# waicool20/BoofCV

Hardware: AMD Instinct MI355X
Metric: 1080p frames/sec detect+describe+associate (higher is better)
Workload: dtype f32 detect / f64 describe / associate: fp16 MFMA candidate filter + exact fp64 re-score; 1 GPU; batch of 256 1920x1080 GrayF32 per GPU: Fast-Hessian detect + SURF-64 (stable) describe + greedy L2 associate with the next frame; batch_per_gpu=256, width=1920, height=1080, ranks_seen=1

## Files before the change

boofcv_amd/csrc/assoc_mfma.hip:

```cpp
#include "common.h"
#include <cfloat>
#include <cmath>
#include <algorithm>

typedef float f32x16 __attribute__((ext_vector_type(16)));
typedef _Float16 h16x8 __attribute__((ext_vector_type(8)));

struct AssocProblem {
	int srcOff, ns, dstOff, nd;
	int rowBase, colBase;
};
struct AssocBlock {
	int p, row0, row1, col0, col1;
};
struct AssocCand {
	int p, i, j, pad;
	double score;
};

#define C16 1.03e-3f
#define ABS16 2.0e-5f
#define BIG16 60000.0f
#define ROW_CHUNKS 9

__device__ __forceinline__ void waveSyncLds() {
	__builtin_amdgcn_fence(__ATOMIC_RELEASE, "wavefront");
	__builtin_amdgcn_wave_barrier();
	__builtin_amdgcn_fence(__ATOMIC_ACQUIRE, "wavefront");
}

__device__ __forceinline__ int scaleExp(float maxN) {
	if (!(maxN > 0.0f)) return 0;
	int e;
	(void)frexpf(maxN, &e);
	return (e + 1) >> 1;
}

#define PREP_ROWS 8
__global__ __launch_bounds__(256) void k_assoc_norms(const double* __restrict__ D, long long rows, float* __restrict__ nrm, int* __restrict__ flags) {
	const long long row0 = (((long long)blockIdx.x * 256 + threadIdx.x) >> 4) * PREP_ROWS;
	const int part = threadIdx.x & 15;
	if (row0 >= rows) return;
	double2 v0[PREP_ROWS], v1[PREP_ROWS];
#pragma unroll
	for (int q = 0; q < PREP_ROWS; q++) {
		const long long row = min(row0 + q, rows - 1);
		const double2* src = (const double2*)(D + row * 64 + 4 * part);
		v0[q] = src[0]; v1[q] = src[1];
	}
#pragma unroll
	for (int q = 0; q < PREP_ROWS; q++) {
		double s = (v0[q].x * v0[q].x + v0[q].y * v0[q].y) + (v1[q].x * v1[q].x + v1[q].y * v1[q].y);
#pragma unroll
		for (int o = 8; o >= 1; o >>= 1) s += __shfl_xor(s, o, 64);
		if (part == 0 && row0 + q < rows) {
			const float n = (float)s;
			const float nUp = n * (1.0f + 4.0f * 5.9604644775390625e-08f);
			nrm[row0 + q] = nUp;
			if (!(s < 1e30)) atomicOr(&flags[0], 1);
			else if (__float_as_int(nUp) > __hip_atomic_load(&flags[1], __ATOMIC_RELAXED, __HIP_MEMORY_SCOPE_AGENT)) atomicMax(&flags[1], __float_as_int(nUp));
		}
	}
}

typedef _Float16 h16x4 __attribute__((ext_vector_type(4)));
__global__ __launch_bounds__(256) void k_assoc_half(const double* __restrict__ D, long long rows, float* __restrict__ nrm, const int* __restrict__ flags,
													  _Float16* __restrict__ Hrow) {
	const long long row0 = (((long long)blockIdx.x * 256 + threadIdx.x) >> 4) * PREP_ROWS;
	const int part = threadIdx.x & 15;
	if (row0 >= rows) return;
	const int q_ = scaleExp(__int_as_float(flags[1]));
	double2 v0[PREP_ROWS], v1[PREP_ROWS];
#pragma unroll
	for (int q = 0; q < PREP_ROWS; q++) {
		const long long row = min(row0 + q, rows - 1);
		const double2* src = (const double2*)(D + row * 64 + 4 * part);
		v0[q] = src[0]; v1[q] = src[1];
	}
#pragma unroll
	for (int q = 0; q < PREP_ROWS; q++) {
		const long long row = row0 + q;
		if (row >= rows) break;
		_Float16* out = Hrow + row * (ROW_CHUNKS * 8);
		const h16x4 hv = {(_Float16)(float)ldexp(v0[q].x, -q_), (_Float16)(float)ldexp(v0[q].y, -q_), (_Float16)(float)ldexp(v1[q].x, -q_),
						  (_Float16)(float)ldexp(v1[q].y, -q_)};
		*(h16x4*)(out + 4 * part) = hv;
		if (part == 0) {
			const float n = ldexpf(nrm[row], -2 * q_);
			const _Float16 hi = (_Float16)n;
			const _Float16 lo = (_Float16)(n - (float)hi);
			const h16x8 e = {hi, lo, (_Float16)1.0f, (_Float16)1.0f, (_Float16)1.0f, (_Float16)0.0f, (_Float16)0.0f, (_Float16)0.0f};
			*(h16x8*)(out + 64) = e;
			nrm[row] = n;
		}
	}
}

__global__ void k_fill_u32(unsigned int* p, long long n, unsigned int v) {
	const long long i = (long long)blockIdx.x * blockDim.x + threadIdx.x;
	if (i < n) p[i] = v;
}

__global__ void k_assoc_thresholds(const AssocProblem* __restrict__ probs, int count, const float* __restrict__ nrmS, const float* __restrict__ nrmD,
								   const unsigned int* __restrict__ rowKey, const unsigned int* __restrict__ colKey, const int* __restrict__ flags,
								   float* __restrict__ rowThr, float* __restrict__ colThr) {
	const int p = blockIdx.y;
	const AssocProblem P = probs[p];
	const float maxRaw = __int_as_float(flags[1]);
	const float maxN = ldexpf(maxRaw, -2 * scaleExp(maxRaw));
	for (int i = blockIdx.x * blockDim.x + threadIdx.x; i < P.ns + P.nd; i += gridDim.x * blockDim.x) {
		if (i < P.ns) {
			const float band = 2.0f * (C16 * (nrmS[P.srcOff + i] + maxN) + ABS16);
			rowThr[P.rowBase + i] = __uint_as_float(rowKey[P.rowBase + i]) + band;
		} else {
			const int j = i - P.ns;
			const float band = 2.0f * (C16 * (nrmD[P.dstOff + j] + maxN) + ABS16);
			colThr[P.colBase + j] = __uint_as_float(colKey[P.colBase + j]) + band;
		}
	}
}

struct MfmaArgs {
	const uint4* Hs;
	const uint4* Hd;
	const AssocProblem* probs;
	const AssocBlock* blocks;
	unsigned int* rowKey;
	unsigned int* colKey;
	const float* rowThr;
	const float* colThr;
	AssocCand* cand;
	int* counter;
	int cap;
#ifdef BHIP_EXPERIMENTS
	int ablate;
#endif
};

#define CAND_LDS 256

__device__ __noinline__ void candSlow(AssocCand* cand, int* counter, int cap, int p, int rr, int col) {
	const int g = atomicAdd(counter, 1);
	if (g < cap) { AssocCand c; c.p = p; c.i = rr; c.j = col; c.pad = 0; c.score = 0; cand[g] = c; }
}
__device__ __forceinline__ void candAdd(const MfmaArgs& A, int2* buf, int* cnt, bool hit, int p, int rr, int col) {
	if (hit) {
		const int pos = atomicAdd(cnt, 1);
		if (pos < CAND_LDS) buf[pos] = make_int2(rr, col);
		else candSlow(A.cand, A.counter, A.cap, p, rr, col);
	}
}
__device__ __forceinline__ void candFlush(const MfmaArgs& A, const int2* buf, const int* cnt, int p, int lane) {
	waveSyncLds();
	const int n = min(*cnt, CAND_LDS);
	if (n == 0) return;
	int base = 0;
	if (lane == 0) base = atomicAdd(A.counter, n);
	base = __builtin_amdgcn_readfirstlane(base);
	for (int k = lane; k < n; k += 64) {
		if (base + k < A.cap) {
			const int2 v = buf[k];
			AssocCand c; c.p = p; c.i = v.x; c.j = v.y; c.pad = 0; c.score = 0;
			A.cand[base + k] = c;
		}
	}
}

__device__ __forceinline__ h16x8 asHalf8(uint4 v) { return __builtin_bit_cast(h16x8, v); }
__device__ __forceinline__ uint4 extChunk(float n0, float n1, float n2, float n3) {
	const h16x8 h = {(_Float16)n0, (_Float16)n1, (_Float16)n2, (_Float16)n3, (_Float16)1.0f, (_Float16)0.0f, (_Float16)0.0f, (_Float16)0.0f};
	return __builtin_bit_cast(uint4, h);
}

#define STRIP_COLS 384
#define STRIP_TILES (STRIP_COLS / 32)
template <int PASS>
__global__ __launch_bounds__(256, 2) void k_assoc_mfma(MfmaArgs A) {
	__shared__ uint4 tileB[STRIP_TILES][10 * 33];
	__shared__ unsigned int colLds[STRIP_COLS];
	__shared__ float rowThrLds[PASS == 2 ? 4 : 1][64];
	__shared__ int2 candLds[PASS == 2 ? 4 : 1][PASS == 2 ? CAND_LDS : 1];
	__shared__ int candCnt[4];
	const AssocBlock B = A.blocks[blockIdx.x];
	if (B.col0 >= B.col1) return;
	const AssocProblem P = A.probs[B.p];
	const int tid = threadIdx.x;
	const int wave = __builtin_amdgcn_readfirstlane(tid >> 6), lane = tid & 63;
	const int r = lane & 31, h = lane >> 5;
	const int ncol = B.col1 - B.col0;
	const int ntile = (ncol + 31) >> 5;
	int2* candBuf = candLds[PASS == 2 ? wave : 0];
	int* candN = &candCnt[wave];
	if (lane == 0) *candN = 0;

	for (int g0 = tid; g0 < ntile * 32 * ROW_CHUNKS; g0 += 4 * 256) {
		uint4 v[4];
#pragma unroll
		for (int q = 0; q < 4; q++) {
			const int g = g0 + 256 * q;
			const int cl = g / ROW_CHUNKS, ch = g - cl * ROW_CHUNKS;
			if (g < ntile * 32 * ROW_CHUNKS && cl < ncol) {
				v[q] = A.Hd[(long long)(P.dstOff + B.col0 + cl) * ROW_CHUNKS + ch];
				if (ch == 8) { const unsigned int x = v[q].x; v[q].x = v[q].y; v[q].y = x; }
			} else {
				v[q] = ch == 8 ? extChunk(1.0f, 1.0f, BIG16, 0.0f) : make_uint4(0, 0, 0, 0);
			}
		}
#pragma unroll
		for (int q = 0; q < 4; q++) {
			const int g = g0 + 256 * q;
			const int cl = g / ROW_CHUNKS, ch = g - cl * ROW_CHUNKS;
			if (g < ntile * 32 * ROW_CHUNKS) tileB[cl >> 5][ch * 33 + (cl & 31)] = v[q];
		}
	}
	for (int g = tid; g < ntile * 32; g += 256) tileB[g >> 5][9 * 33 + (g & 31)] = make_uint4(0, 0, 0, 0);
	for (int c = tid; c < ntile * 32; c += 256)
		colLds[c] = PASS == 1 ? 0xFFFFFFFFu : (c < ncol ? __float_as_uint(A.colThr[P.colBase + B.col0 + c]) : __float_as_uint(-INFINITY));
	__syncthreads();

	uint4 araw[2][5];
	auto loadA = [&](int rowT) {
#pragma unroll
		for (int t = 0; t < 2; t++) {
			const int row = rowT + 32 * t + r;
			if (row < B.row1) {
				const uint4* src = A.Hs + (long long)(P.srcOff + row) * ROW_CHUNKS;
#pragma unroll
				for (int s = 0; s < 4; s++) araw[t][s] = src[2 * s + h];
				araw[t][4] = h == 0 ? src[8] : make_uint4(0, 0, 0, 0);
			} else {
#pragma unroll
				for (int s = 0; s < 4; s++) araw[t][s] = make_uint4(0, 0, 0, 0);
				araw[t][4] = h == 0 ? extChunk(BIG16, 0.0f, 1.0f, 1.0f) : make_uint4(0, 0, 0, 0);
			}
		}
	};
	if (B.row0 + 64 * wave < B.row1) loadA(B.row0 + 64 * wave);
	for (int rowT = B.row0 + 64 * wave; rowT < B.row1; rowT += 256) {
		h16x8 a[2][5];
#pragma unroll
		for (int t = 0; t < 2; t++) {
#pragma unroll
			for (int s = 0; s < 4; s++) a[t][s] = asHalf8(araw[t][s]) * (_Float16)(-2.0f);
			a[t][4] = asHalf8(araw[t][4]);
		}
		if (rowT + 256 < B.row1 && !BHIP_ABLATE(A, 4)) loadA(rowT + 256);
		unsigned int rowM[32];
#pragma unroll
		for (int k = 0; k < 32; k++) rowM[k] = 0xFFFFFFFFu;
		if (PASS == 2) {
			waveSyncLds();
			rowThrLds[wave][lane] = rowT + lane < B.row1 ? A.rowThr[P.rowBase + rowT + lane] : -INFINITY;
			waveSyncLds();
		}
		for (int ct = 0; ct < ntile; ct += 2) {
			const bool two = ct + 1 < ntile;
			const int cA_ = 32 * ct + r, cB_ = cA_ + 32;
			f32x16 acc[2][2];
#pragma unroll
			for (int t = 0; t < 2; t++)
#pragma unroll
				for (int c = 0; c < 2; c++)
#pragma unroll
					for (int g = 0; g < 16; g++) acc[t][c][g] = (c == 0 || two) ? 0.0f : INFINITY;
#pragma unroll
			for (int s = 0; s < 5 && !BHIP_ABLATE(A, 1); s++) {
				const int ch = s < 4 ? 2 * s + h : 8 + h;
				const h16x8 b0 = asHalf8(tileB[ct][ch * 33 + r]);
				acc[0][0] = __builtin_amdgcn_mfma_f32_32x32x16_f16(a[0][s], b0, acc[0][0], 0, 0, 0);
				acc[1][0] = __builtin_amdgcn_mfma_f32_32x32x16_f16(a[1][s], b0, acc[1][0], 0, 0, 0);
				if (two) {
					const h16x8 b1 = asHalf8(tileB[ct + 1][ch * 33 + r]);
					acc[0][1] = __builtin_amdgcn_mfma_f32_32x32x16_f16(a[0][s], b1, acc[0][1], 0, 0, 0);
					acc[1][1] = __builtin_amdgcn_mfma_f32_32x32x16_f16(a[1][s], b1, acc[1][1], 0, 0, 0);
				}
			}
			if (BHIP_ABLATE(A, 2)) continue;
			if (PASS == 1) {
				unsigned int cA = 0xFFFFFFFFu, cB = 0xFFFFFFFFu;
// ... 83 lines not shown
		atomicMin(&colBest[P.colBase + c->j], bits);
	}
}

__global__ __launch_bounds__(256) void k_assoc_argsel(const AssocProblem* __restrict__ probs, const AssocCand* __restrict__ cand,
														const int* __restrict__ counter, int cap, const unsigned long long* __restrict__ rowBest,
														const unsigned long long* __restrict__ colBest, int* __restrict__ rowArg, int* __restrict__ colArg,
														int* __restrict__ colCnt) {
	const int n = min(*counter, cap);
	for (int t = blockIdx.x * blockDim.x + threadIdx.x; t < n; t += gridDim.x * blockDim.x) {
		const AssocCand c = cand[t];
		const AssocProblem P = probs[c.p];
		const unsigned long long bits = (unsigned long long)__double_as_longlong(c.score);
		if (bits == rowBest[P.rowBase + c.i]) atomicMax(&rowArg[P.rowBase + c.i], c.j);
		if (bits == colBest[P.colBase + c.j]) {
			atomicAdd(&colCnt[P.colBase + c.j], 1);
			atomicMax(&colArg[P.colBase + c.j], c.i);
		}
	}
}

__global__ __launch_bounds__(256) void k_assoc_resolve(const AssocProblem* __restrict__ probs, double maxErr, int backwards,
														 const unsigned long long* __restrict__ rowBest, const int* __restrict__ rowArg,
														 const int* __restrict__ colArg, const int* __restrict__ colCnt, int* __restrict__ pairs,
														 double* __restrict__ fit) {
	const AssocProblem P = probs[blockIdx.y];
	for (int i = blockIdx.x * blockDim.x + threadIdx.x; i < P.ns; i += gridDim.x * blockDim.x) {
		const int m = rowArg[P.rowBase + i];
		const double best = __longlong_as_double((long long)rowBest[P.rowBase + i]);
		int outPair = -1;
		double outFit = maxErr;
		if (m >= 0 && best <= maxErr) {
			outPair = m;
			outFit = best;
			if (backwards) {
				if (!(colArg[P.colBase + m] == i && colCnt[P.colBase + m] == 1)) { outPair = -1; outFit = DBL_MAX; }
			}
		}
		pairs[P.srcOff + i] = outPair;
		fit[P.srcOff + i] = outFit;
	}
}

int bhip_assoc_l2_mfma_batched(bhip_ctx* ctx, AssocMfmaWork& W, const double* dev_src, const double* dev_dst, int count, const long long* srcOff,
								 const int* ns, const long long* dstOff, const int* nd, double maxErr, int backwards, int* dev_pairs, double* dev_fit,
								 int* usedMfma) {
	*usedMfma = 0;
	if (count <= 0) { *usedMfma = 1; return BHIP_OK; }
	std::vector<AssocProblem> probs(count);
	std::vector<AssocBlock> blocks;
	long long maxSrcRow = 0, maxDstRow = 0, rowTotal = 0, colTotal = 0;
	double flopsPerPass = 0;
	for (int p = 0; p < count; p++) {
		if (ns[p] <= 0 || nd[p] <= 0) return BHIP_OK;
		if (srcOff[p] + ns[p] > 0x7fffffffLL || dstOff[p] + nd[p] > 0x7fffffffLL) return BHIP_OK;
		probs[p] = {(int)srcOff[p], ns[p], (int)dstOff[p], nd[p], (int)rowTotal, (int)colTotal};
		maxSrcRow = std::max(maxSrcRow, srcOff[p] + ns[p]);
		maxDstRow = std::max(maxDstRow, dstOff[p] + nd[p]);
		rowTotal += ns[p];
		colTotal += nd[p];
		flopsPerPass += 2.0 * ns[p] * (double)nd[p] * 64;
		if (rowTotal > 0x3fffffffLL || colTotal > 0x3fffffffLL) return BHIP_OK;
	}
	long long strips = 0;
	for (int p = 0; p < count; p++) strips += (nd[p] + STRIP_COLS - 1) / STRIP_COLS;
	int rowSplit = (int)std::max<long long>(1, (1024 + strips - 1) / strips);
	{ const char* e = getenv("BHIP_ASSOC_ROWSPLIT"); if (e && atoi(e) > 0) rowSplit = atoi(e); }
	for (int p = 0; p < count; p++) {
		int chunk = (ns[p] + rowSplit - 1) / rowSplit;
		chunk = std::max(256, ((chunk + 255) / 256) * 256);
		for (int c0 = 0; c0 < nd[p]; c0 += STRIP_COLS)
			for (int r0 = 0; r0 < ns[p]; r0 += chunk) blocks.push_back({p, r0, std::min(ns[p], r0 + chunk), c0, std::min(nd[p], c0 + STRIP_COLS)});
	}
	if (count >= 16) {
		std::vector<AssocBlock> q[8];
		for (const AssocBlock& b : blocks) q[b.p & 7].push_back(b);
		size_t longest = 0;
		for (int x = 0; x < 8; x++) longest = std::max(longest, q[x].size());
		blocks.assign(longest * 8, AssocBlock{0, 0, 0, 0, 0});
		for (int x = 0; x < 8; x++)
			for (size_t k = 0; k < q[x].size(); k++) blocks[k * 8 + x] = q[x][k];
	}
	const bool shared = dev_src == dev_dst;
	const long long rowsS = shared ? std::max(maxSrcRow, maxDstRow) : maxSrcRow;
	const int cap = (int)std::min<long long>(0x3fffffffLL, 8 * (rowTotal + colTotal) + 4096);

	BHIP_TRY(W.Fs.reserve(ctx, (size_t)rowsS * ROW_CHUNKS * 16));
	BHIP_TRY(W.nrmS.reserve(ctx, (size_t)rowsS * 4));
	if (!shared) {
		BHIP_TRY(W.Fd.reserve(ctx, (size_t)maxDstRow * ROW_CHUNKS * 16));
		BHIP_TRY(W.nrmD.reserve(ctx, (size_t)maxDstRow * 4));
	}
	BHIP_TRY(W.probs.reserve(ctx, probs.size() * sizeof(AssocProblem)));
	BHIP_TRY(W.blocks.reserve(ctx, blocks.size() * sizeof(AssocBlock)));
	BHIP_TRY(W.keys.reserve(ctx, (size_t)(rowTotal + colTotal) * 4));
	BHIP_TRY(W.thr.reserve(ctx, (size_t)(rowTotal + colTotal) * 4));
	BHIP_TRY(W.best.reserve(ctx, (size_t)(rowTotal + colTotal) * 8));
	BHIP_TRY(W.args.reserve(ctx, (size_t)(rowTotal + 2 * colTotal) * 4));
	BHIP_TRY(W.cand.reserve(ctx, (size_t)cap * sizeof(AssocCand)));
	BHIP_TRY(W.flags.reserve(ctx, 64));

	hipStream_t st = ctx->stream;
	BHIP_HIP(ctx, hipMemcpyAsync(W.probs.p, probs.data(), probs.size() * sizeof(AssocProblem), hipMemcpyHostToDevice, st));
	BHIP_HIP(ctx, hipMemcpyAsync(W.blocks.p, blocks.data(), blocks.size() * sizeof(AssocBlock), hipMemcpyHostToDevice, st));
	BHIP_HIP(ctx, hipMemsetAsync(W.flags.p, 0, 64, st));
	int* flags = W.flags.as<int>();
	int* counters = flags + 2;
	_Float16* Hs = W.Fs.as<_Float16>();
	float* nS = W.nrmS.as<float>();
	_Float16* Hd = shared ? Hs : W.Fd.as<_Float16>();
	float* nD = shared ? nS : W.nrmD.as<float>();
	{
		ProfScope ps(ctx, "k_assoc_prep", (double)(rowsS + (shared ? 0 : maxDstRow)) * (2 * 64 * 8 + ROW_CHUNKS * 16));
		const unsigned gS = (unsigned)((rowsS + 16 * PREP_ROWS - 1) / (16 * PREP_ROWS)), gD = (unsigned)((maxDstRow + 16 * PREP_ROWS - 1) / (16 * PREP_ROWS));
		hipLaunchKernelGGL(k_assoc_norms, dim3(gS), dim3(256), 0, st, dev_src, rowsS, nS, flags);
		if (!shared) hipLaunchKernelGGL(k_assoc_norms, dim3(gD), dim3(256), 0, st, dev_dst, maxDstRow, nD, flags);
		hipLaunchKernelGGL(k_assoc_half, dim3(gS), dim3(256), 0, st, dev_src, rowsS, nS, flags, Hs);
		if (!shared) hipLaunchKernelGGL(k_assoc_half, dim3(gD), dim3(256), 0, st, dev_dst, maxDstRow, nD, flags, Hd);
	}
	unsigned int* rowKey = W.keys.as<unsigned int>();
	unsigned int* colKey = rowKey + rowTotal;
	float* rowThr = W.thr.as<float>();
	float* colThr = rowThr + rowTotal;
	unsigned long long* rowBest = W.best.as<unsigned long long>();
	unsigned long long* colBest = rowBest + rowTotal;
	int* rowArg = W.args.as<int>();
	int* colArg = rowArg + rowTotal;
	int* colCnt = colArg + colTotal;
	const long long nk = rowTotal + colTotal;
	hipLaunchKernelGGL(k_fill_u32, dim3((unsigned)((nk + 255) / 256)), dim3(256), 0, st, rowKey, nk, 0xFFFFFFFFu);
	BHIP_HIP(ctx, hipMemsetAsync(W.best.p, 0xFF, (size_t)nk * 8, st));
	BHIP_HIP(ctx, hipMemsetAsync(rowArg, 0xFF, (size_t)(rowTotal + colTotal) * 4, st));
	BHIP_HIP(ctx, hipMemsetAsync(colCnt, 0, (size_t)colTotal * 4, st));

	MfmaArgs A;
	A.Hs = (const uint4*)Hs; A.Hd = (const uint4*)Hd; A.probs = W.probs.as<AssocProblem>(); A.blocks = W.blocks.as<AssocBlock>();
	A.rowKey = rowKey; A.colKey = colKey; A.rowThr = rowThr; A.colThr = colThr;
	A.cand = W.cand.as<AssocCand>(); A.counter = counters; A.cap = cap;
#ifdef BHIP_EXPERIMENTS
	{ const char* e = getenv("BHIP_ASSOC_ABLATE"); A.ablate = e ? atoi(e) : 0; }
#endif
	const unsigned nblocks = (unsigned)blocks.size();
	{
		ProfScope ps(ctx, "k_assoc_mfma_pass1", 0, flopsPerPass);
		hipLaunchKernelGGL(k_assoc_mfma<1>, dim3(nblocks), dim3(256), 0, st, A);
	}
	int maxN = 0;
	for (int p = 0; p < count; p++) maxN = std::max(maxN, ns[p] + nd[p]);
	hipLaunchKernelGGL(k_assoc_thresholds, dim3((maxN + 255) / 256, count), dim3(256), 0, st, A.probs, count, nS, nD, rowKey, colKey, flags, rowThr, colThr);
	{
		ProfScope ps(ctx, "k_assoc_mfma_pass2", 0, flopsPerPass);
		hipLaunchKernelGGL(k_assoc_mfma<2>, dim3(nblocks), dim3(256), 0, st, A);
	}
	{
		ProfScope ps(ctx, "k_assoc_exact");
		const unsigned exactBlocks = (unsigned)std::min<long long>(16384, std::max<long long>(256, (3 * (rowTotal + colTotal) / 2 + 255) / 256));
		hipLaunchKernelGGL(k_assoc_exact, dim3(exactBlocks), dim3(256), 0, st, dev_src, dev_dst, A.probs, A.cand, counters, cap, rowBest, colBest);
		hipLaunchKernelGGL(k_assoc_argsel, dim3(exactBlocks), dim3(256), 0, st, A.probs, A.cand, counters, cap, rowBest, colBest, rowArg, colArg, colCnt);
	}
	BHIP_HIP(ctx, hipMemcpyAsync(ctx->hostScratch.p, flags, 16, hipMemcpyDeviceToHost, st));
	BHIP_HIP(ctx, hipStreamSynchronize(st));
	const int* hf = ctx->hostScratch.as<int>();
	if (hf[0] != 0 || hf[2] > cap) return BHIP_OK;
	int maxNs = 0;
	for (int p = 0; p < count; p++) maxNs = std::max(maxNs, ns[p]);
	hipLaunchKernelGGL(k_assoc_resolve, dim3((maxNs + 255) / 256, count), dim3(256), 0, st, A.probs, maxErr, backwards, rowBest, rowArg, colArg, colCnt,
					   dev_pairs, dev_fit);
	BHIP_HIP(ctx, hipGetLastError());
	*usedMfma = 1;
	return BHIP_OK;
}
```

boofcv_amd/csrc/cabi.hip:

```cpp
#include "cabi.h"

HandleRegistry& registry() {
	static HandleRegistry* r = [] {
		HandleRegistry* p = new HandleRegistry();
		atexit([] { registry().exiting = true; });
		return p;
	}();
	return *r;
}

static int ctxCreate(int device, void* stream, bool useGiven, bhip_ctx** out) {
	if (!out) return BHIP_ERR_INVALID;
	*out = nullptr;
	int count = 0;
	if (hipGetDeviceCount(&count) != hipSuccess || count <= 0) return BHIP_ERR_HIP;
	if (device < 0 || device >= count) return BHIP_ERR_INVALID;
	if (hipSetDevice(device) != hipSuccess) return BHIP_ERR_HIP;
	std::unique_ptr<bhip_ctx_full> ctx(new (std::nothrow) bhip_ctx_full());
	if (!ctx) return BHIP_ERR_NOMEM;
	ctx->device = device;
	if (hipDeviceGetAttribute(&ctx->cuCount, hipDeviceAttributeMultiprocessorCount, device) != hipSuccess || ctx->cuCount <= 0) return BHIP_ERR_HIP;
	if (useGiven) {
		ctx->stream = (hipStream_t)stream;
	} else {
// ... 15 lines not shown
struct FhOctavePlan {
	int skip, w, h, nlevels;
	int sizes[BHIP_MAX_LEVELS];
	std::vector<FhLevelPlan> mids;
	bool fused = false, fixed = false;
	int shareFrom[BHIP_MAX_LEVELS];
	bool onDemand[BHIP_MAX_LEVELS];
	int exportSlot[BHIP_MAX_LEVELS];
	int nexport = 0;
	size_t intenOff = 0, expOff = 0;
	long long intenImageStride = 0, expImageStride = 0;
};

struct FhDetector {
	bhip_fh_cfg cfg;
	int W = 0, H = 0, batch = 0, cap = 0;
	bool plannedInt = false;
	std::vector<FhOctavePlan> plan;
	int bitmapWords = 0;
	DevBuf inten, bitmap, prefix, cand, sorted, count, selKey, selIdx, selLevels;
	bool nBest() const { return cfg.maxFeaturesPerScale > 0; }
	std::vector<int> counts;
	long long total = 0;

	static bool unfusedOnly() { return bhip_env_flag("BHIP_DETECT_UNFUSED"); }
	int makePlan(bhip_ctx* ctx, int width, int height) {
		plan.clear();
		if (cfg.numberScalesPerOctave > BHIP_MAX_LEVELS || cfg.numberScalesPerOctave < 1) return bhip_fail(ctx, BHIP_ERR_UNSUPPORTED, "numberScalesPerOctave out of range");
		if (cfg.extractRadius < 1) return bhip_fail(ctx, BHIP_ERR_INVALID, "Search radius must be >= 1");
		if (cfg.initialSampleSize < 1 || cfg.initialSize < 3) return bhip_fail(ctx, BHIP_ERR_INVALID, "bad sample size / initial size");
		if (width >= 32768 || height >= 32768) return bhip_fail(ctx, BHIP_ERR_UNSUPPORTED, "image too large for Point2D_I16");
		int skip = cfg.initialSampleSize, sizeStep = cfg.scaleStepSize, octaveSize = cfg.initialSize;
		unsigned int bits = 0;
		const int step = cfg.extractRadius + 1;
		for (int octave = 0; octave < cfg.numberOfOctaves; octave++) {
			FhOctavePlan o;
			o.nlevels = cfg.numberScalesPerOctave;
			for (int i = 0; i < o.nlevels; i++) o.sizes[i] = octaveSize + i * sizeStep;
			const int maxSize = o.sizes[o.nlevels - 1];
			if (maxSize > width || maxSize > height) break;
			o.skip = skip;
			o.w = width / skip;
			o.h = height / skip;
			for (int i = 2; i < o.nlevels; i++) {
				FhLevelPlan m;
				m.level = i - 1;
// ... 142 lines not shown
					FusedExport ex{0, {0, 0}, nullptr, 0, 0, 0, {0, 0}};
					if (o.nexport > 0 && k + 1 < plan.size()) {
						const FhOctavePlan& c = plan[k + 1];
						ex.n = o.nexport;
						for (int j = 0; j < o.nlevels; j++) if (o.exportSlot[j] >= 0) ex.level[o.exportSlot[j]] = j;
						ex.out = level(c, 0).data; ex.w = c.w; ex.h = c.h; ex.imageStride = c.intenImageStride;
						for (int i = 0; i < c.nlevels; i++) {
							const int j = c.shareFrom[i];
							if (j >= 0 && o.exportSlot[j] >= 0) ex.slotOffset[o.exportSlot[j]] = (long long)i * c.w * c.h;
						}
					}
					BHIP_TRY(bhip_launch_detect_fused(ctx, ii, o.skip, o.nlevels, o.sizes, (int)o.mids.size(), mp, ml, cfg.extractRadius,
													  cfg.detectThreshold, bitmap.as<unsigned int>(), bitmapWords, cand.as<KeyPoint>(), count.as<int>(), cap,
													  ex.n > 0 ? &ex : nullptr));
					continue;
				}
				size_t end = k + 1;
				while (!nBest() && end < plan.size() && !plan[end].fused) end++;
				BHIP_TRY(runStandAlone(ctx, ii, k, end));
				k = end - 1;
			}
			BHIP_TRY(bhip_launch_word_prefix(ctx, bitmap.as<unsigned int>(), bitmapWords, batch, prefix.as<unsigned int>(), count.as<int>() + batch));
			counts.resize(batch);
			if ((size_t)batch * 4 <= (1u << 20)) {
				BHIP_HIP(ctx, hipMemcpyAsync(ctx->hostScratch.p, count.p, (size_t)batch * 4, hipMemcpyDeviceToHost, ctx->stream));
				BHIP_HIP(ctx, hipStreamSynchronize(ctx->stream));
				memcpy(counts.data(), ctx->hostScratch.p, (size_t)batch * 4);
			} else {
				BHIP_HIP(ctx, hipMemcpyAsync(counts.data(), count.p, (size_t)batch * 4, hipMemcpyDeviceToHost, ctx->stream));
				BHIP_HIP(ctx, hipStreamSynchronize(ctx->stream));
			}
			int maxCount = 0;
			total = 0;
			for (int c : counts) { maxCount = std::max(maxCount, c); total += c; }
			if (maxCount <= cap) {
				BHIP_TRY(bhip_launch_rank_scatter(ctx, bitmap.as<unsigned int>(), bitmapWords, prefix.as<unsigned int>(), cand.as<KeyPoint>(), count.as<int>(),
												  cap, batch, sorted.as<KeyPoint>()));
				if (nBest()) BHIP_TRY(selectNBest(ctx));
				return BHIP_OK;
			}
			cap = maxCount + maxCount / 4 + 64;
			BHIP_TRY(allocate(ctx));
		}
		return bhip_fail(ctx, BHIP_ERR_CAPACITY, "key point list kept overflowing");
	}
	int selectNBest(bhip_ctx* ctx) {
		int nlv = 0;
		for (auto& o : plan) nlv += (int)o.mids.size();
		int* levelStart = selLevels.as<int>();
		int* levelCount = levelStart + (size_t)std::max(nlv, 1) * batch;
		int li = 0;
		for (auto& o : plan)
			for (auto& m : o.mids) {
				BHIP_TRY(bhip_launch_select_nbest(ctx, level(o, m.level - 1), level(o, m.level), level(o, m.level + 1), m.p, cfg.extractRadius,
												  cfg.maxFeaturesPerScale, bitmap.as<unsigned int>(), prefix.as<unsigned int>(), bitmapWords, sorted.as<KeyPoint>(),
												  cap, selKey.as<float>(), selIdx.as<int>(), cand.as<KeyPoint>(), levelStart, levelCount, li, nlv));
				li++;
			}
		BHIP_TRY(bhip_launch_compact_levels(ctx, cand.as<KeyPoint>(), cap, levelStart, levelCount, nlv, batch, sorted.as<KeyPoint>(), count.as<int>()));
		BHIP_HIP(ctx, hipMemcpyAsync(counts.data(), count.p, (size_t)batch * 4, hipMemcpyDeviceToHost, ctx->stream));
		BHIP_HIP(ctx, hipStreamSynchronize(ctx->stream));
// ... 698 lines not shown
```

boofcv_amd/csrc/common.h:

```cpp
#pragma once
#include <hip/hip_runtime.h>
#include <cstdint>
#include <cstdio>
#include <cstring>
#include <cstdlib>
#include <string>
#include <type_traits>
#include <vector>
#include <new>
#include <utility>
#include "../../include/boofhip.h"

#define BHIP_WAVE 64

static inline bool bhip_env_flag(const char* name) {
	const char* e = getenv(name);
	return e && e[0] == '1';
}
#ifdef BHIP_EXPERIMENTS
#define BHIP_ABLATE(P, bits) ((P).ablate & (bits))
#else
#define BHIP_ABLATE(P, bits) 0
#endif

// ... 73 lines not shown
	DevBuf(DevBuf&& o) noexcept : p(o.p), cap(o.cap) { o.p = nullptr; o.cap = 0; }
	DevBuf& operator=(DevBuf&& o) noexcept { std::swap(p, o.p); std::swap(cap, o.cap); return *this; }
	~DevBuf() { if (p) (void)hipFree(p); }
	int reserve(bhip_ctx* ctx, size_t bytes) {
		if (bytes <= cap) return BHIP_OK;
		if (p) { BHIP_HIP(ctx, hipStreamSynchronize(ctx->stream)); BHIP_HIP(ctx, hipFree(p)); p = nullptr; cap = 0; }
		size_t want = bytes + bytes / 8;
		BHIP_HIP(ctx, hipMalloc(&p, want));
		cap = want;
		return BHIP_OK;
	}
	template <class T> T* as() const { return (T*)p; }
};

inline int PinnedBuf::reserve(bhip_ctx* ctx, size_t bytes) {
	if (bytes <= cap) return BHIP_OK;
	if (p) { BHIP_HIP(ctx, hipStreamSynchronize(ctx->stream)); (void)hipHostFree(p); p = nullptr; cap = 0; }
	if (hipHostMalloc(&p, bytes, hipHostMallocDefault) != hipSuccess) { (void)hipGetLastError(); p = nullptr; return bhip_fail(ctx, BHIP_ERR_NOMEM, "page-locked staging buffer"); }
	cap = bytes;
	return BHIP_OK;
}

struct AssocMfmaWork {
	DevBuf Fs, Fd, nrmS, nrmD, probs, blocks, keys, thr, best, args, cand, flags;
};

struct ImgView {
	const float* data;
	long long imageStride;
	int stride;
	int width, height;
};
struct ImgViewW {
	float* data;
	long long imageStride;
	int stride;
	int width, height;
};

template <class T>
struct DevImg {
	T* data;
	long long imageStride;
	int stride, width, height, batch;
	operator DevImg<const T>() const { return {data, imageStride, stride, width, height, batch}; }
};
template <class T>
// ... 380 lines not shown
```

boofcv_amd/csrc/detect.hip:

```cpp
#include "hessian_dev.h"
#include <cfloat>

template <bool MIN> __device__ __forceinline__ bool nmsBeats(float a, float b) { return MIN ? a <= b : a >= b; }
template <bool MIN> __device__ __forceinline__ float nmsPad() { return MIN ? INFINITY : -INFINITY; }
template <bool MIN> __device__ __forceinline__ float nmsMarker() { return MIN ? -FLT_MAX : FLT_MAX; }
template <int RT, bool MIN = false>
__device__ __forceinline__ bool strictLocalMax(const float* __restrict__ img, int stride, int w, int h, int x, int y, int r, float v, float thr) {
	if (!nmsBeats<MIN>(v, thr) || v == nmsMarker<MIN>()) return false;
	bool isMax = true;
	if (RT > 0) {
		float nb[(2 * RT + 1) * (2 * RT + 1)];
#pragma unroll
		for (int j = -RT; j <= RT; j++)
#pragma unroll
			for (int i = -RT; i <= RT; i++) {
				const int xx = x + i, yy = y + j;
				const bool in = xx >= 0 && xx < w && yy >= 0 && yy < h && !(i == 0 && j == 0);
				nb[(j + RT) * (2 * RT + 1) + i + RT] = in ? img[(long long)yy * stride + xx] : nmsPad<MIN>();
			}
#pragma unroll
		for (int k = 0; k < (2 * RT + 1) * (2 * RT + 1); k++)
			if (nmsBeats<MIN>(nb[k], v)) isMax = false;
	} else {
		const int x0 = max(x - r, 0), x1 = min(x + r, w - 1), y0 = max(y - r, 0), y1 = min(y + r, h - 1);
// ... 330 lines not shown
}

int bhip_launch_word_prefix(bhip_ctx* ctx, const unsigned int* bitmap, int bitmapWords, int batch, unsigned int* wordPrefix, int* totals) {
	if (batch <= 0 || bitmapWords <= 0) return BHIP_OK;
	{
		ProfScope ps(ctx, "k_word_prefix", 8.0 * bitmapWords * batch);
		hipLaunchKernelGGL(k_word_prefix, dim3(batch), dim3(1024), 0, ctx->stream, bitmap, bitmapWords, wordPrefix, totals);
	}
	BHIP_HIP(ctx, hipGetLastError());
	return BHIP_OK;
}

__global__ __launch_bounds__(256) void k_rank_scatter(const unsigned int* __restrict__ bitmap, int words, const unsigned int* __restrict__ prefix,
													   const KeyPoint* __restrict__ cand, const int* __restrict__ candCount, int cap,
													   KeyPoint* __restrict__ sorted) {
	const int img = blockIdx.y;
	const int n = min(candCount[img], cap);
	const int i = blockIdx.x * blockDim.x + threadIdx.x;
	if (i >= n) return;
	const KeyPoint kp = cand[(long long)img * cap + i];
	const unsigned int word = kp.key >> 5, bit = kp.key & 31;
	const unsigned int below = bitmap[(long long)img * words + word] & ((1u << bit) - 1u);
	const unsigned int rank = prefix[(long long)img * words + word] + __popc(below);
	sorted[(long long)img * cap + rank] = kp;
}

int bhip_launch_rank_scatter(bhip_ctx* ctx, const unsigned int* bitmap, int bitmapWords, unsigned int* wordPrefix, const KeyPoint* cand,
							 const int* candCount, int cap, int batch, KeyPoint* sorted) {
	if (batch <= 0 || cap <= 0) return BHIP_OK;
	dim3 grid((cap + 255) / 256, batch);
	{
		ProfScope ps(ctx, "k_rank_scatter");
		hipLaunchKernelGGL(k_rank_scatter, grid, dim3(256), 0, ctx->stream, bitmap, bitmapWords, (const unsigned int*)wordPrefix, cand, candCount, cap, sorted);
	}
	BHIP_HIP(ctx, hipGetLastError());
	return BHIP_OK;
}

#define SEL_LDS 4096

struct SelectParams {
	const float* lower;
	const float* mid;
	const float* upper;
	long long imageStride;
	int stride;
	DetectLevelParams p;
// ... 385 lines not shown
```

Before: 16190 frames/s.

## Speculate fp16 scale from previous call and fold assoc prep/init launches

The association path now guesses the fp16 scaling exponent from the previous call. This lets norms and fp16 conversion fuse into one prep kernel, and the result is validated afterwards, re-running the whole association if the guess was wrong. Memsets, fills and host-to-device table copies are folded into a single init kernel that copies the tables from pinned host memory. The threshold kernel is removed by computing thresholds inside pass 2, and resolve is launched before the host sync and gated on device flags. Detection overlaps rank-scatter with the count readback, the MFMA loop peels the odd tail tile, and a mispredicted scale costs a full second run.

```diff
diff --git a/boofcv_amd/csrc/assoc_mfma.hip b/boofcv_amd/csrc/assoc_mfma.hip
--- a/boofcv_amd/csrc/assoc_mfma.hip
+++ b/boofcv_amd/csrc/assoc_mfma.hip
@@ -1,6 +1,7 @@
 #include "common.h"
 #include <cfloat>
 #include <cmath>
+#include <cstring>
 #include <algorithm>
 
 typedef float f32x16 __attribute__((ext_vector_type(16)));
@@ -29,11 +30,22 @@
 	__builtin_amdgcn_fence(__ATOMIC_ACQUIRE, "wavefront");
 }
 
-__device__ __forceinline__ int scaleExp(float maxN) {
+__host__ __device__ __forceinline__ int scaleExp(float maxN) {
 	if (!(maxN > 0.0f)) return 0;
 	int e;
 	(void)frexpf(maxN, &e);
 	return (e + 1) >> 1;
+}
+__host__ __device__ __forceinline__ bool scaleHolds(float maxN, int q) {
+	if (!(maxN > 0.0f)) return true;
+	int e;
+	(void)frexpf(maxN, &e);
+	return e >= 2 * q - 3 && e <= 2 * q;
+}
+__host__ __device__ __forceinline__ bool assocDegenerate(const int* flags, int cap) {
+	float maxN;
+	memcpy(&maxN, &flags[1], 4);
+	return flags[0] != 0 || flags[2] > cap || !scaleHolds(maxN, flags[3]);
 }
 
 #define PREP_ROWS 8
@@ -64,12 +76,13 @@
 }
 
 typedef _Float16 h16x4 __attribute__((ext_vector_type(4)));
-__global__ __launch_bounds__(256) void k_assoc_half(const double* __restrict__ D, long long rows, float* __restrict__ nrm, const int* __restrict__ flags,
+__global__ __launch_bounds__(256) void k_assoc_half(const double* __restrict__ D, long long rows, float* __restrict__ nrm, int* __restrict__ flags,
 													  _Float16* __restrict__ Hrow) {
 	const long long row0 = (((long long)blockIdx.x * 256 + threadIdx.x) >> 4) * PREP_ROWS;
 	const int part = threadIdx.x & 15;
 	if (row0 >= rows) return;
 	const int q_ = scaleExp(__int_as_float(flags[1]));
+	if (blockIdx.x == 0 && threadIdx.x == 0) flags[3] = q_;
 	double2 v0[PREP_ROWS], v1[PREP_ROWS];
 #pragma unroll
 	for (int q = 0; q < PREP_ROWS; q++) {
@@ -96,28 +109,55 @@
 	}
 }
 
-__global__ void k_fill_u32(unsigned int* p, long long n, unsigned int v) {
-	const long long i = (long long)blockIdx.x * blockDim.x + threadIdx.x;
-	if (i < n) p[i] = v;
-}
-
-__global__ void k_assoc_thresholds(const AssocProblem* __restrict__ probs, int count, const float* __restrict__ nrmS, const float* __restrict__ nrmD,
-								   const unsigned int* __restrict__ rowKey, const unsigned int* __restrict__ colKey, const int* __restrict__ flags,
-								   float* __restrict__ rowThr, float* __restrict__ colThr) {
-	const int p = blockIdx.y;
-	const AssocProblem P = probs[p];
-	const float maxRaw = __int_as_float(flags[1]);
-	const float maxN = ldexpf(maxRaw, -2 * scaleExp(maxRaw));
-	for (int i = blockIdx.x * blockDim.x + threadIdx.x; i < P.ns + P.nd; i += gridDim.x * blockDim.x) {
-		if (i < P.ns) {
-			const float band = 2.0f * (C16 * (nrmS[P.srcOff + i] + maxN) + ABS16);
-			rowThr[P.rowBase + i] = __uint_as_float(rowKey[P.rowBase + i]) + band;
-		} else {
-			const int j = i - P.ns;
-			const float band = 2.0f * (C16 * (nrmD[P.dstOff + j] + maxN) + ABS16);
-			colThr[P.colBase + j] = __uint_as_float(colKey[P.colBase + j]) + band;
-		}
-	}
+__global__ __launch_bounds__(256) void k_assoc_prep_hinted(const double* __restrict__ D, long long rows, int q_, float* __restrict__ nrm, int* __restrict__ flags,
+															 _Float16* __restrict__ Hrow) {
+	const long long row0 = (((long long)blockIdx.x * 256 + threadIdx.x) >> 4) * PREP_ROWS;
+	const int part = threadIdx.x & 15;
+	if (row0 >= rows) return;
+	double2 v0[PREP_ROWS], v1[PREP_ROWS];
+#pragma unroll
+	for (int q = 0; q < PREP_ROWS; q++) {
+		const long long row = min(row0 + q, rows - 1);
+		const double2* src = (const double2*)(D + row * 64 + 4 * part);
+		v0[q] = src[0]; v1[q] = src[1];
+	}
+#pragma unroll
+	for (int q = 0; q < PREP_ROWS; q++) {
+		double s = (v0[q].x * v0[q].x + v0[q].y * v0[q].y) + (v1[q].x * v1[q].x + v1[q].y * v1[q].y);
+#pragma unroll
+		for (int o = 8; o >= 1; o >>= 1) s += __shfl_xor(s, o, 64);
+		const long long row = row0 + q;
+		if (row >= rows) continue;
+		_Float16* out = Hrow + row * (ROW_CHUNKS * 8);
+		const h16x4 hv = {(_Float16)(float)ldexp(v0[q].x, -q_), (_Float16)(float)ldexp(v0[q].y, -q_), (_Float16)(float)ldexp(v1[q].x, -q_),
+						  (_Float16)(float)ldexp(v1[q].y, -q_)};
+		*(h16x4*)(out + 4 * part) = hv;
+		if (part == 0) {
+			const float nRaw = (float)s;
+			const float nUp = nRaw * (1.0f + 4.0f * 5.9604644775390625e-08f);
+			if (!(s < 1e30)) atomicOr(&flags[0], 1);
+			else if (__float_as_int(nUp) > __hip_atomic_load(&flags[1], __ATOMIC_RELAXED, __HIP_MEMORY_SCOPE_AGENT)) atomicMax(&flags[1], __float_as_int(nUp));
+			const float n = ldexpf(nUp, -2 * q_);
+			const _Float16 hi = (_Float16)n;
+			const _Float16 lo = (_Float16)(n - (float)hi);
+			const h16x8 e = {hi, lo, (_Float16)1.0f, (_Float16)1.0f, (_Float16)1.0f, (_Float16)0.0f, (_Float16)0.0f, (_Float16)0.0f};
+			*(h16x8*)(out + 64) = e;
+			nrm[row] = n;
+		}
+	}
+}
+
+__global__ __launch_bounds__(256) void k_assoc_init(unsigned int* __restrict__ keys, unsigned long long* __restrict__ best, int* __restrict__ args, long long nk,
+													  long long colTotal, int* __restrict__ flags, int q_, const uint4* __restrict__ tabSrc, uint4* __restrict__ tabDst,
+													  long long tabWords) {
+	const long long i = (long long)blockIdx.x * 256 + threadIdx.x;
+	if (i < tabWords) tabDst[i] = tabSrc[i];
+	if (i < 16) flags[i] = i == 3 ? q_ : 0;
+	if (i >= nk) return;
+	keys[i] = 0xFFFFFFFFu;
+	best[i] = ~0ull;
+	args[i] = -1;
+	if (i < colTotal) args[nk + i] = 0;
 }
 
 struct MfmaArgs {
@@ -127,8 +167,9 @@
 	const AssocBlock* blocks;
 	unsigned int* rowKey;
 	unsigned int* colKey;
-	const float* rowThr;
-	const float* colThr;
+	const float* nrmS;
+	const float* nrmD;
+	const int* flags;
 	AssocCand* cand;
 	int* counter;
 	int cap;
@@ -172,6 +213,9 @@
 	return __builtin_bit_cast(uint4, h);
 }
 
+#ifndef BHIP_ASSOC_PEEL
+#define BHIP_ASSOC_PEEL 1
+#endif
 #define STRIP_COLS 384
 #define STRIP_TILES (STRIP_COLS / 32)
 template <int PASS>
@@ -214,8 +258,20 @@
 		}
 	}
 	for (int g = tid; g < ntile * 32; g += 256) tileB[g >> 5][9 * 33 + (g & 31)] = make_uint4(0, 0, 0, 0);
-	for (int c = tid; c < ntile * 32; c += 256)
-		colLds[c] = PASS == 1 ? 0xFFFFFFFFu : (c < ncol ? __float_as_uint(A.colThr[P.colBase + B.col0 + c]) : __float_as_uint(-INFINITY));
+	float maxN = 0.0f;
+	if (PASS == 2) maxN = ldexpf(__int_as_float(A.flags[1]), -2 * A.flags[3]);
+	for (int c = tid; c < ntile * 32; c += 256) {
+		unsigned int v = 0xFFFFFFFFu;
+		if (PASS == 2) {
+			float thr = -INFINITY;
+			if (c < ncol) {
+				const float band = 2.0f * (C16 * (A.nrmD[P.dstOff + B.col0 + c] + maxN) + ABS16);
+				thr = __uint_as_float(A.colKey[P.colBase + B.col0 + c]) + band;
+			}
+			v = __float_as_uint(thr);
+		}
+		colLds[c] = v;
+	}
 	__syncthreads();
 
 	uint4 araw[2][5];
@@ -250,11 +306,18 @@
 		for (int k = 0; k < 32; k++) rowM[k] = 0xFFFFFFFFu;
 		if (PASS == 2) {
 			waveSyncLds();
-			rowThrLds[wave][lane] = rowT + lane < B.row1 ? A.rowThr[P.rowBase + rowT + lane] : -INFINITY;
+			float thr = -INFINITY;
+			if (rowT + lane < B.row1) {
+				const float band = 2.0f * (C16 * (A.nrmS[P.srcOff + rowT + lane] + maxN) + ABS16);
+				thr = __uint_as_float(A.rowKey[P.rowBase + rowT + lane]) + band;
+			}
+			rowThrLds[wave][lane] = thr;
 			waveSyncLds();
 		}
-		for (int ct = 0; ct < ntile; ct += 2) {
-			const bool two = ct + 1 < ntile;
+#pragma unroll
+		for (int round = 0; round <= BHIP_ASSOC_PEEL; round++)
+		for (int ct = round == 0 ? 0 : (ntile & ~1); ct < (BHIP_ASSOC_PEEL && round == 0 ? (ntile & ~1) : ntile); ct += 2) {
+			const bool two = BHIP_ASSOC_PEEL ? round == 0 : ct + 1 < ntile;
 			const int cA_ = 32 * ct + r, cB_ = cA_ + 32;
 			f32x16 acc[2][2];
 #pragma unroll
@@ -384,8 +447,9 @@
 
 __global__ __launch_bounds__(256) void k_assoc_resolve(const AssocProblem* __restrict__ probs, double maxErr, int backwards,
 														 const unsigned long long* __restrict__ rowBest, const int* __restrict__ rowArg,
-														 const int* __restrict__ colArg, const int* __restrict__ colCnt, int* __restrict__ pairs,
-														 double* __restrict__ fit) {
+														 const int* __restrict__ colArg, const int* __restrict__ colCnt, const int* __restrict__ flags, int cap,
+														 int* __restrict__ pairs, double* __restrict__ fit) {
+	if (assocDegenerate(flags, cap)) return;
 	const AssocProblem P = probs[blockIdx.y];
 	for (int i = blockIdx.x * blockDim.x + threadIdx.x; i < P.ns; i += gridDim.x * blockDim.x) {
 		const int m = rowArg[P.rowBase + i];
@@ -424,25 +488,27 @@
 		flopsPerPass += 2.0 * ns[p] * (double)nd[p] * 64;
 		if (rowTotal > 0x3fffffffLL || colTotal > 0x3fffffffLL) return BHIP_OK;
 	}
-	long long strips = 0;
-	for (int p = 0; p < count; p++) strips += (nd[p] + STRIP_COLS - 1) / STRIP_COLS;
-	int rowSplit = (int)std::max<long long>(1, (1024 + strips - 1) / strips);
-	{ const char* e = getenv("BHIP_ASSOC_ROWSPLIT"); if (e && atoi(e) > 0) rowSplit = atoi(e); }
-	for (int p = 0; p < count; p++) {
-		int chunk = (ns[p] + rowSplit - 1) / rowSplit;
-		chunk = std::max(256, ((chunk + 255) / 256) * 256);
-		for (int c0 = 0; c0 < nd[p]; c0 += STRIP_COLS)
-			for (int r0 = 0; r0 < ns[p]; r0 += chunk) blocks.push_back({p, r0, std::min(ns[p], r0 + chunk), c0, std::min(nd[p], c0 + STRIP_COLS)});
-	}
-	if (count >= 16) {
-		std::vector<AssocBlock> q[8];
-		for (const AssocBlock& b : blocks) q[b.p & 7].push_back(b);
-		size_t longest = 0;
-		for (int x = 0; x < 8; x++) longest = std::max(longest, q[x].size());
-		blocks.assign(longest * 8, AssocBlock{0, 0, 0, 0, 0});
-		for (int x = 0; x < 8; x++)
-			for (size_t k = 0; k < q[x].size(); k++) blocks[k * 8 + x] = q[x][k];
-	}
+	auto buildBlocks = [&]() {
+		long long strips = 0;
+		for (int p = 0; p < count; p++) strips += (nd[p] + STRIP_COLS - 1) / STRIP_COLS;
+		int rowSplit = (int)std::max<long long>(1, (1024 + strips - 1) / strips);
+		{ const char* e = getenv("BHIP_ASSOC_ROWSPLIT"); if (e && atoi(e) > 0) rowSplit = atoi(e); }
+		for (int p = 0; p < count; p++) {
+			int chunk = (ns[p] + rowSplit - 1) / rowSplit;
+			chunk = std::max(256, ((chunk + 255) / 256) * 256);
+			for (int c0 = 0; c0 < nd[p]; c0 += STRIP_COLS)
+				for (int r0 = 0; r0 < ns[p]; r0 += chunk) blocks.push_back({p, r0, std::min(ns[p], r0 + chunk), c0, std::min(nd[p], c0 + STRIP_COLS)});
+		}
+		if (count >= 16) {
+			std::vector<AssocBlock> q[8];
+			for (const AssocBlock& b : blocks) q[b.p & 7].push_back(b);
+			size_t longest = 0;
+			for (int x = 0; x < 8; x++) longest = std::max(longest, q[x].size());
+			blocks.assign(longest * 8, AssocBlock{0, 0, 0, 0, 0});
+			for (int x = 0; x < 8; x++)
+				for (size_t k = 0; k < q[x].size(); k++) blocks[k * 8 + x] = q[x][k];
+		}
+	};
 	const bool shared = dev_src == dev_dst;
 	const long long rowsS = shared ? std::max(maxSrcRow, maxDstRow) : maxSrcRow;
 	const int cap = (int)std::min<long long>(0x3fffffffLL, 8 * (rowTotal + colTotal) + 4096);
@@ -453,82 +519,102 @@
 		BHIP_TRY(W.Fd.reserve(ctx, (size_t)maxDstRow * ROW_CHUNKS * 16));
 		BHIP_TRY(W.nrmD.reserve(ctx, (size_t)maxDstRow * 4));
 	}
-	BHIP_TRY(W.probs.reserve(ctx, probs.size() * sizeof(AssocProblem)));
-	BHIP_TRY(W.blocks.reserve(ctx, blocks.size() * sizeof(AssocBlock)));
 	BHIP_TRY(W.keys.reserve(ctx, (size_t)(rowTotal + colTotal) * 4));
-	BHIP_TRY(W.thr.reserve(ctx, (size_t)(rowTotal + colTotal) * 4));
 	BHIP_TRY(W.best.reserve(ctx, (size_t)(rowTotal + colTotal) * 8));
 	BHIP_TRY(W.args.reserve(ctx, (size_t)(rowTotal + 2 * colTotal) * 4));
 	BHIP_TRY(W.cand.reserve(ctx, (size_t)cap * sizeof(AssocCand)));
 	BHIP_TRY(W.flags.reserve(ctx, 64));
 
 	hipStream_t st = ctx->stream;
-	BHIP_HIP(ctx, hipMemcpyAsync(W.probs.p, probs.data(), probs.size() * sizeof(AssocProblem), hipMemcpyHostToDevice, st));
-	BHIP_HIP(ctx, hipMemcpyAsync(W.blocks.p, blocks.data(), blocks.size() * sizeof(AssocBlock), hipMemcpyHostToDevice, st));
-	BHIP_HIP(ctx, hipMemsetAsync(W.flags.p, 0, 64, st));
 	int* flags = W.flags.as<int>();
 	int* counters = flags + 2;
 	_Float16* Hs = W.Fs.as<_Float16>();
 	float* nS = W.nrmS.as<float>();
 	_Float16* Hd = shared ? Hs : W.Fd.as<_Float16>();
 	float* nD = shared ? nS : W.nrmD.as<float>();
-	{
-		ProfScope ps(ctx, "k_assoc_prep", (double)(rowsS + (shared ? 0 : maxDstRow)) * (2 * 64 * 8 + ROW_CHUNKS * 16));
-		const unsigned gS = (unsigned)((rowsS + 16 * PREP_ROWS - 1) / (16 * PREP_ROWS)), gD = (unsigned)((maxDstRow + 16 * PREP_ROWS - 1) / (16 * PREP_ROWS));
-		hipLaunchKernelGGL(k_assoc_norms, dim3(gS), dim3(256), 0, st, dev_src, rowsS, nS, flags);
-		if (!shared) hipLaunchKernelGGL(k_assoc_norms, dim3(gD), dim3(256), 0, st, dev_dst, maxDstRow, nD, flags);
-		hipLaunchKernelGGL(k_assoc_half, dim3(gS), dim3(256), 0, st, dev_src, rowsS, nS, flags, Hs);
-		if (!shared) hipLaunchKernelGGL(k_assoc_half, dim3(gD), dim3(256), 0, st, dev_dst, maxDstRow, nD, flags, Hd);
-	}
 	unsigned int* rowKey = W.keys.as<unsigned int>();
 	unsigned int* colKey = rowKey + rowTotal;
-	float* rowThr = W.thr.as<float>();
-	float* colThr = rowThr + rowTotal;
 	unsigned long long* rowBest = W.best.as<unsigned long long>();
 	unsigned long long* colBest = rowBest + rowTotal;
 	int* rowArg = W.args.as<int>();
 	int* colArg = rowArg + rowTotal;
 	int* colCnt = colArg + colTotal;
 	const long long nk = rowTotal + colTotal;
-	hipLaunchKernelGGL(k_fill_u32, dim3((unsigned)((nk + 255) / 256)), dim3(256), 0, st, rowKey, nk, 0xFFFFFFFFu);
-	BHIP_HIP(ctx, hipMemsetAsync(W.best.p, 0xFF, (size_t)nk * 8, st));
-	BHIP_HIP(ctx, hipMemsetAsync(rowArg, 0xFF, (size_t)(rowTotal + colTotal) * 4, st));
-	BHIP_HIP(ctx, hipMemsetAsync(colCnt, 0, (size_t)colTotal * 4, st));
+	int maxNs = 0;
+	for (int p = 0; p < count; p++) maxNs = std::max(maxNs, ns[p]);
+	const size_t blocksAt = (probs.size() * sizeof(AssocProblem) + 15) & ~(size_t)15;
 
 	MfmaArgs A;
-	A.Hs = (const uint4*)Hs; A.Hd = (const uint4*)Hd; A.probs = W.probs.as<AssocProblem>(); A.blocks = W.blocks.as<AssocBlock>();
-	A.rowKey = rowKey; A.colKey = colKey; A.rowThr = rowThr; A.colThr = colThr;
+	A.Hs = (const uint4*)Hs; A.Hd = (const uint4*)Hd;
+	A.rowKey = rowKey; A.colKey = colKey; A.nrmS = nS; A.nrmD = nD; A.flags = flags;
 	A.cand = W.cand.as<AssocCand>(); A.counter = counters; A.cap = cap;
 #ifdef BHIP_EXPERIMENTS
 	{ const char* e = getenv("BHIP_ASSOC_ABLATE"); A.ablate = e ? atoi(e) : 0; }
 #endif
+	const unsigned gS = (unsigned)((rowsS + 16 * PREP_ROWS - 1) / (16 * PREP_ROWS)), gD = (unsigned)((maxDstRow + 16 * PREP_ROWS - 1) / (16 * PREP_ROWS));
+	const double prepRows = (double)(rowsS + (shared ? 0 : maxDstRow));
+
+	buildBlocks();
+	const size_t tableBytes = (blocksAt + blocks.size() * sizeof(AssocBlock) + 15) & ~(size_t)15;
+	BHIP_TRY(W.probs.reserve(ctx, tableBytes));
+	if (W.tablesInFlight) { BHIP_HIP(ctx, hipStreamSynchronize(st)); W.tablesInFlight = false; }
+	if (tableBytes > W.tables.cap) BHIP_TRY(W.tables.reserve(ctx, tableBytes * 2));
+	memcpy(W.tables.p, probs.data(), probs.size() * sizeof(AssocProblem));
+	memcpy((char*)W.tables.p + blocksAt, blocks.data(), blocks.size() * sizeof(AssocBlock));
+	void* tablesDev = nullptr;
+	BHIP_HIP(ctx, hipHostGetDevicePointer(&tablesDev, W.tables.p, 0));
+	if (!W.flagsRead) BHIP_HIP(ctx, hipEventCreateWithFlags(&W.flagsRead.h, hipEventDisableTiming));
+	A.probs = W.probs.as<AssocProblem>();
+	A.blocks = (const AssocBlock*)((const char*)W.probs.p + blocksAt);
 	const unsigned nblocks = (unsigned)blocks.size();
-	{
-		ProfScope ps(ctx, "k_assoc_mfma_pass1", 0, flopsPerPass);
-		hipLaunchKernelGGL(k_assoc_mfma<1>, dim3(nblocks), dim3(256), 0, st, A);
-	}
-	int maxN = 0;
-	for (int p = 0; p < count; p++) maxN = std::max(maxN, ns[p] + nd[p]);
-	hipLaunchKernelGGL(k_assoc_thresholds, dim3((maxN + 255) / 256, count), dim3(256), 0, st, A.probs, count, nS, nD, rowKey, colKey, flags, rowThr, colThr);
-	{
-		ProfScope ps(ctx, "k_assoc_mfma_pass2", 0, flopsPerPass);
-		hipLaunchKernelGGL(k_assoc_mfma<2>, dim3(nblocks), dim3(256), 0, st, A);
-	}
-	{
-		ProfScope ps(ctx, "k_assoc_exact");
-		const unsigned exactBlocks = (unsigned)std::min<long long>(16384, std::max<long long>(256, (3 * (rowTotal + colTotal) / 2 + 255) / 256));
-		hipLaunchKernelGGL(k_assoc_exact, dim3(exactBlocks), dim3(256), 0, st, dev_src, dev_dst, A.probs, A.cand, counters, cap, rowBest, colBest);
-		hipLaunchKernelGGL(k_assoc_argsel, dim3(exactBlocks), dim3(256), 0, st, A.probs, A.cand, counters, cap, rowBest, colBest, rowArg, colArg, colCnt);
-	}
-	BHIP_HIP(ctx, hipMemcpyAsync(ctx->hostScratch.p, flags, 16, hipMemcpyDeviceToHost, st));
-	BHIP_HIP(ctx, hipStreamSynchronize(st));
-	const int* hf = ctx->hostScratch.as<int>();
-	if (hf[0] != 0 || hf[2] > cap) return BHIP_OK;
-	int maxNs = 0;
-	for (int p = 0; p < count; p++) maxNs = std::max(maxNs, ns[p]);
-	hipLaunchKernelGGL(k_assoc_resolve, dim3((maxNs + 255) / 256, count), dim3(256), 0, st, A.probs, maxErr, backwards, rowBest, rowArg, colArg, colCnt,
-					   dev_pairs, dev_fit);
-	BHIP_HIP(ctx, hipGetLastError());
-	*usedMfma = 1;
+
+	for (int run = 0; run < 2; run++) {
+		const bool hinted = run == 0;
+		const long long tabWords = hinted ? (long long)(tableBytes / 16) : 0;
+		W.tablesInFlight = true;
+		hipLaunchKernelGGL(k_assoc_init, dim3((unsigned)((std::max(nk, tabWords) + 255) / 256)), dim3(256), 0, st, rowKey, rowBest, rowArg, nk, colTotal, flags,
+						   hinted ? W.scaleHint : 0, (const uint4*)tablesDev, W.probs.as<uint4>(), tabWords);
+		if (hinted) {
+			ProfScope ps(ctx, "k_assoc_prep", prepRows * (64 * 8 + ROW_CHUNKS * 16));
+			hipLaunchKernelGGL(k_assoc_prep_hinted, dim3(gS), dim3(256), 0, st, dev_src, rowsS, W.scaleHint, nS, flags, Hs);
+			if (!shared) hipLaunchKernelGGL(k_assoc_prep_hinted, dim3(gD), dim3(256), 0, st, dev_dst, maxDstRow, W.scaleHint, nD, flags, Hd);
+		} else {
+			ProfScope ps(ctx, "k_assoc_prep", prepRows * (2 * 64 * 8 + ROW_CHUNKS * 16));
+			hipLaunchKernelGGL(k_assoc_norms, dim3(gS), dim3(256), 0, st, dev_src, rowsS, nS, flags);
+			if (!shared) hipLaunchKernelGGL(k_assoc_norms, dim3(gD), dim3(256), 0, st, dev_dst, maxDstRow, nD, flags);
+			hipLaunchKernelGGL(k_assoc_half, dim3(gS), dim3(256), 0, st, dev_src, rowsS, nS, flags, Hs);
+			if (!shared) hipLaunchKernelGGL(k_assoc_half, dim3(gD), dim3(256), 0, st, dev_dst, maxDstRow, nD, flags, Hd);
+		}
+		{
+			ProfScope ps(ctx, "k_assoc_mfma_pass1", 0, flopsPerPass);
+			hipLaunchKernelGGL(k_assoc_mfma<1>, dim3(nblocks), dim3(256), 0, st, A);
+		}
+		{
+			ProfScope ps(ctx, "k_assoc_mfma_pass2", 0, flopsPerPass);
+			hipLaunchKernelGGL(k_assoc_mfma<2>, dim3(nblocks), dim3(256), 0, st, A);
+		}
+		{
+			ProfScope ps(ctx, "k_assoc_exact");
+			const unsigned exactBlocks = (unsigned)std::min<long long>(16384, std::max<long long>(256, (3 * (rowTotal + colTotal) / 2 + 255) / 256));
+			hipLaunchKernelGGL(k_assoc_exact, dim3(exactBlocks), dim3(256), 0, st, dev_src, dev_dst, A.probs, A.cand, counters, cap, rowBest, colBest);
+			hipLaunchKernelGGL(k_assoc_argsel, dim3(exactBlocks), dim3(256), 0, st, A.probs, A.cand, counters, cap, rowBest, colBest, rowArg, colArg, colCnt);
+		}
+		BHIP_HIP(ctx, hipMemcpyAsync(ctx->hostScratch.p, flags, 16, hipMemcpyDeviceToHost, st));
+		BHIP_HIP(ctx, hipEventRecord(W.flagsRead, st));
+		hipLaunchKernelGGL(k_assoc_resolve, dim3((maxNs + 255) / 256, count), dim3(256), 0, st, A.probs, maxErr, backwards, rowBest, rowArg, colArg, colCnt,
+						   flags, cap, dev_pairs, dev_fit);
+		BHIP_HIP(ctx, hipEventSynchronize(W.flagsRead));
+		W.tablesInFlight = false;
+		BHIP_HIP(ctx, hipGetLastError());
+		const int* hf = ctx->hostScratch.as<int>();
+		if (hf[0] != 0) return BHIP_OK;
+		float maxRaw;
+		memcpy(&maxRaw, &hf[1], 4);
+		if (maxRaw > 0.0f) W.scaleHint = scaleExp(maxRaw);
+		if (!scaleHolds(maxRaw, hf[3])) continue;
+		if (hf[2] > cap) return BHIP_OK;
+		*usedMfma = 1;
+		return BHIP_OK;
+	}
 	return BHIP_OK;
 }
diff --git a/boofcv_amd/csrc/cabi.hip b/boofcv_amd/csrc/cabi.hip
--- a/boofcv_amd/csrc/cabi.hip
+++ b/boofcv_amd/csrc/cabi.hip
@@ -61,6 +61,7 @@
 	bool nBest() const { return cfg.maxFeaturesPerScale > 0; }
 	std::vector<int> counts;
 	long long total = 0;
+	HipEvent countsRead;
 
 	static bool unfusedOnly() { return bhip_env_flag("BHIP_DETECT_UNFUSED"); }
 	int makePlan(bhip_ctx* ctx, int width, int height) {
@@ -249,21 +250,27 @@
 			}
 			BHIP_TRY(bhip_launch_word_prefix(ctx, bitmap.as<unsigned int>(), bitmapWords, batch, prefix.as<unsigned int>(), count.as<int>() + batch));
 			counts.resize(batch);
-			if ((size_t)batch * 4 <= (1u << 20)) {
-				BHIP_HIP(ctx, hipMemcpyAsync(ctx->hostScratch.p, count.p, (size_t)batch * 4, hipMemcpyDeviceToHost, ctx->stream));
-				BHIP_HIP(ctx, hipStreamSynchronize(ctx->stream));
-				memcpy(counts.data(), ctx->hostScratch.p, (size_t)batch * 4);
+			const bool viaScratch = (size_t)batch * 4 <= (1u << 20);
+			BHIP_HIP(ctx, hipMemcpyAsync(viaScratch ? ctx->hostScratch.p : (void*)counts.data(), count.p, (size_t)batch * 4, hipMemcpyDeviceToHost, ctx->stream));
+			if (!nBest()) {
+				if (!countsRead) BHIP_HIP(ctx, hipEventCreateWithFlags(&countsRead.h, hipEventDisableTiming));
+				BHIP_HIP(ctx, hipEventRecord(countsRead, ctx->stream));
+				BHIP_TRY(bhip_launch_rank_scatter(ctx, bitmap.as<unsigned int>(), bitmapWords, prefix.as<unsigned int>(), cand.as<KeyPoint>(), count.as<int>(),
+												  cap, batch, sorted.as<KeyPoint>()));
+				BHIP_HIP(ctx, hipEventSynchronize(countsRead));
 			} else {
-				BHIP_HIP(ctx, hipMemcpyAsync(counts.data(), count.p, (size_t)batch * 4, hipMemcpyDeviceToHost, ctx->stream));
 				BHIP_HIP(ctx, hipStreamSynchronize(ctx->stream));
 			}
+			if (viaScratch) memcpy(counts.data(), ctx->hostScratch.p, (size_t)batch * 4);
 			int maxCount = 0;
 			total = 0;
 			for (int c : counts) { maxCount = std::max(maxCount, c); total += c; }
 			if (maxCount <= cap) {
-				BHIP_TRY(bhip_launch_rank_scatter(ctx, bitmap.as<unsigned int>(), bitmapWords, prefix.as<unsigned int>(), cand.as<KeyPoint>(), count.as<int>(),
-												  cap, batch, sorted.as<KeyPoint>()));
-				if (nBest()) BHIP_TRY(selectNBest(ctx));
+				if (nBest()) {
+					BHIP_TRY(bhip_launch_rank_scatter(ctx, bitmap.as<unsigned int>(), bitmapWords, prefix.as<unsigned int>(), cand.as<KeyPoint>(), count.as<int>(),
+													  cap, batch, sorted.as<KeyPoint>()));
+					BHIP_TRY(selectNBest(ctx));
+				}
 				return BHIP_OK;
 			}
 			cap = maxCount + maxCount / 4 + 64;
diff --git a/boofcv_amd/csrc/common.h b/boofcv_amd/csrc/common.h
--- a/boofcv_amd/csrc/common.h
+++ b/boofcv_amd/csrc/common.h
@@ -119,7 +119,11 @@
 }
 
 struct AssocMfmaWork {
-	DevBuf Fs, Fd, nrmS, nrmD, probs, blocks, keys, thr, best, args, cand, flags;
+	DevBuf Fs, Fd, nrmS, nrmD, probs, keys, best, args, cand, flags;
+	PinnedBuf tables;
+	bool tablesInFlight = false;
+	HipEvent flagsRead;
+	int scaleHint = 1;
 };
 
 struct ImgView {
diff --git a/boofcv_amd/csrc/detect.hip b/boofcv_amd/csrc/detect.hip
--- a/boofcv_amd/csrc/detect.hip
+++ b/boofcv_amd/csrc/detect.hip
@@ -376,7 +376,7 @@
 	const unsigned int word = kp.key >> 5, bit = kp.key & 31;
 	const unsigned int below = bitmap[(long long)img * words + word] & ((1u << bit) - 1u);
 	const unsigned int rank = prefix[(long long)img * words + word] + __popc(below);
-	sorted[(long long)img * cap + rank] = kp;
+	if (rank < (unsigned int)cap) sorted[(long long)img * cap + rank] = kp;
 }
 
 int bhip_launch_rank_scatter(bhip_ctx* ctx, const unsigned int* bitmap, int bitmapWords, unsigned int* wordPrefix, const KeyPoint* cand,
```

New measurement: 16370 frames/s, median of 6. +1.1%, better.
